# google-research/FirstOrderLp.jl

Hardware: AMD Instinct MI355X
Metric: pdhg_iterations_per_sec (higher is better)
Workload: dtype f64; 1 GPU; random LP m=10000000 n=10000000 nnz=100000000 seed=12345 (BASELINE configs[4]), adaptive step, zero start, no restarts/rescaling; id=configs[4], m=10000000, n=10000000, nnz=100000000, parallelism=single GPU

## Files before the change

firstorderlp.jl_amd/csrc/abi_batch.hpp:

```cpp

struct BatchProduct {
  int rows = 0, grid = 0, slots = 0, long_thr = 0;
  int nlong = 0, nchunks = 0, long_grid = 0, chunk_grid = 0;
  int *long_row = nullptr, *long_cptr = nullptr;
  int2 *chunks = nullptr;
  double *cpart = nullptr;
  double *part = nullptr;
};

struct BatchState {
  int K = 0, shift = 0;
  std::vector<pdhg_handle *> mem;
  BatchProduct PA, PT;
  double *X = nullptr, *Y = nullptr;
  BatchMemberDev *mdev = nullptr, *mhost = nullptr;
  int *act_dev = nullptr, *act_host = nullptr;
  double *res_dev = nullptr, *res_host = nullptr;
  int64_t trials = 0;
};

static void batch_free_product(BatchProduct &P) {
  for (void *p : {(void *)P.long_row, (void *)P.long_cptr, (void *)P.chunks, (void *)P.cpart, (void *)P.part})
    if (p) (void)hipFree(p);
  P = BatchProduct{};
// ... 60 lines not shown
    HIP_TRY(hipMemcpy(P.long_cptr, lcptr.data(), sizeof(int) * lcptr.size(), hipMemcpyHostToDevice));
    HIP_TRY(hipMemcpy(P.chunks, ch.data(), sizeof(int2) * ch.size(), hipMemcpyHostToDevice));
    int rc = alloc_zero(&P.cpart, (int64_t)P.nchunks << shift);
    if (rc) return rc;
  }
  P.slots = P.grid + P.long_grid;
  return 0;
}

static pdhg_handle *batch_of(pdhg_handle *h) { return (h && h->bat) ? h : nullptr; }

static int batch_scale_members(pdhg_handle *h, const double *dv, const double *ev) {
  for (pdhg_handle *m : h->bat->mem) {
    hipLaunchKernelGGL(batch_scale_vectors_kernel, dim3(h->ew_grid_nm), dim3(TPB), 0, h->stream, (int)h->n, (int)h->m, dv, ev,
                       m->c, m->lb, m->ub, m->b);
    m->state_version += 1;
    m->matrix_version += 1;
  }
  HIP_TRY(hipGetLastError());
  return 0;
}

int pdhg_create_batch(pdhg_handle **out, int count, int64_t m, int64_t n, int64_t nnz, const int64_t *colptr,
                      const int64_t *rowval, const double *nzval, int index_base, const double *c, const double *b,
                      const double *lb, const double *ub, int64_t num_equalities, int device_id, void *stream) {
  if (!out) return fail(-1, "out == NULL");
  *out = nullptr;
  if (count < 1 || count > BATCH_MAX) return fail(-1, "pdhg_create_batch: count must be 1.." + std::to_string(BATCH_MAX));
  if (!c || !lb || !ub || (m > 0 && !b)) return fail(-1, "null input array");
  int64_t cap = (int64_t)INT32_MAX - 1;
// ... 175 lines not shown
```

firstorderlp.jl_amd/csrc/abi_measure.hpp:

```cpp


int pdhg_profile_enable(pdhg_handle *h, int enable) {
  int rc0 = check_handle(h);
  if (rc0) return rc0;
  h->profile = enable != 0;
  if (enable) for (int k = 0; k < PDHG_K_COUNT; ++k) { h->prof_count[k] = 0; h->prof_ms[k] = 0.0; }
  return 0;
}

int pdhg_profile_read(pdhg_handle *h, int kernel_id, int64_t *launches, double *total_ms) {
  if (!h || kernel_id < 0 || kernel_id >= PDHG_K_COUNT) return fail(-1, "bad kernel id");
  *launches = h->prof_count[kernel_id];
  *total_ms = h->prof_ms[kernel_id];
  return 0;
}

int64_t pdhg_kernel_algorithmic_bytes(pdhg_handle *h, int kernel_id) {
  if (!h) return -1;
  const int64_t m = h->m, n = h->n, nnz = h->nnz, cn = h->cn;
  const bool group = h->grp != nullptr;
  switch (kernel_id) {
    case PDHG_K_PRIMAL: return 8 * (7 + (h->lazy_accept ? 2 : 0)) * cn;
    case PDHG_K_SPMV_DUAL:
      return nnz * 12 + (m + 1) * 4 + n * 8 + (3 + (h->lazy_accept ? 2 : 0)) * m * 8;
// ... 316 lines not shown

int pdhg_layout_describe(pdhg_handle *h, char *buf, int cap) {
  if (!h) return fail(-1, "null handle");
  std::string out = "{\"A\": " + describe_matrix(h, h->A, MODE_DUAL, 0) + ", \"At\": " + describe_matrix(h, h->At, h->grp ? MODE_PLAIN : MODE_ATY, 1);
  if (h->has_q) out += ", \"Q\": " + describe_matrix(h, h->Q, MODE_PLAIN, 2) + ", \"Qt\": " + describe_matrix(h, h->Qt, MODE_PLAIN, 2);
  if (h->grp && !h->Achunk.empty()) {
    char b[256];
    snprintf(b, sizeof b, ", \"all_gather\": {\"chunks\": %d, \"mode\": \"%s\", \"columns_per_rank_and_chunk\": %lld, \"passes\": [",
             (int)h->Achunk.size(), (h->grp->ag_mode == 1 && h->grp->backend == COMM_RCCL) ? "overlapped with A_p xbar" : "passes behind one all-gather",
             (long long)h->grp->ag_sub);
    out += b;
    for (size_t c = 0; c < h->Achunk.size(); ++c)
      out += (c ? ", " : "") + describe_matrix(h, h->Achunk[c], c + 1 < h->Achunk.size() ? MODE_PLAIN : MODE_DUAL, 0);
    out += "]}";
  }
  const char *tv = getenv("PDHG_TUNE");
  out += std::string(", \"row_order\": \"") + (h->relaxed ? "relaxed" : "strict") + "\", \"timing_at_create\": " + ((tv && tv[0] == '0') ? "false" : "true") + "}";
  if (buf && cap > 0) {
    const size_t k = std::min(out.size(), (size_t)cap - 1);
    memcpy(buf, out.data(), k);
    buf[k] = 0;
  }
  return (int)out.size();
}

int pdhg_layout_info(pdhg_handle *h, int64_t info[16]) {
  if (!h) return fail(-1, "null handle");
  info[12] = (int64_t)h->A.slabs.size(); info[13] = (int64_t)h->At.slabs.size();
  info[14] = (coop_eligible(h) || h->coop_mode == 1) ? 2 : ((graph_eligible(h) || (h->graph_mode == 1 && !h->has_q)) ? 1 : 0);
  info[15] = ((h->A.tiled && h->A.var_tiles) || (!h->A.segs.empty() && h->A.segs.front().tiled && h->A.segs.front().var_tiles) ? 1 : 0) +
// ... 31 lines not shown
```

firstorderlp.jl_amd/csrc/abi_rescale.hpp:

```cpp


static int row_grid(int rows) { return std::max(1, (rows + (TPB / WAVE) - 1) / (TPB / WAVE)); }

struct RescaleTmp {
  double *ev = nullptr, *dv = nullptr, *inv_e = nullptr, *inv_d = nullptr, *cum_e = nullptr, *cum_d = nullptr;
  double *tmp_e = nullptr, *tmp_d = nullptr;
};

extern "C++" {
template <int OP>
static void launch_row_op(pdhg_handle *h, const CsrDev &D, int cols, double pexp, const double *inv_scale, double *out) {
  if (!D.segs.empty()) {
    for (const CsrDev &S : D.segs) launch_row_op<OP>(h, S, cols, pexp, inv_scale ? inv_scale + S.row0 : inv_scale, out + S.row0);
    return;
  }
  hipLaunchKernelGGL(row_op_kernel<OP>, dim3(row_grid(D.rows)), dim3(TPB), 0, h->stream, D.view(), cols, pexp, inv_scale, out,
                     D.long_thr);
  if (D.nlong > 0) {
    hipLaunchKernelGGL(row_op_long_partial_kernel<OP>, dim3(D.nchunks), dim3(TPB), 0, h->stream, D.view(),
                       (const int *)D.chunk_row, (const int *)D.chunk_off, pexp, inv_scale, D.chunk_partial);
    hipLaunchKernelGGL(row_op_long_final_kernel<OP>, dim3(D.long_grid), dim3(TPB), 0, h->stream, D.view(),
                       (const int *)D.long_row, (const int *)D.long_chunk_ptr, D.nlong,
                       (const double *)D.chunk_partial, cols, pexp, out);
  }
// ... 34 lines not shown
  scale_one(h->At, t.inv_e, t.inv_d, 1);
  if (!h->Achunk.empty() && h->grp) {
    DistGroup &g = *h->grp;
    int rc2 = launch_chunk_pack(g, t.inv_d, h->xchunk, 0, g.world, h->n, h->stream);
    if (rc2) return rc2;
    const int64_t W = (int64_t)g.world * g.ag_sub;
    for (size_t c = 0; c < h->Achunk.size(); ++c) scale_one(h->Achunk[c], t.inv_e, h->xchunk + (int64_t)c * W, 0);
  }
  if (h->has_q) {
    scale_one(h->Q, t.inv_d, t.inv_d, 0);
    scale_one(h->Qt, t.inv_d, t.inv_d, 1);
  }
  hipLaunchKernelGGL(resc_apply_vectors_kernel, dim3(h->ew_grid_nm), dim3(TPB), 0, h->stream, n, m, t.dv, t.ev,
                     h->c, h->lb, h->ub, h->b, t.cum_d, t.cum_e);
  HIP_TRY(hipGetLastError());
  if (h->bat) return batch_scale_members(h, t.dv, t.ev);
  return 0;
}

int pdhg_rescale(pdhg_handle *h0, int l_inf_ruiz_iterations, int l2_norm_rescaling,
                 int use_pock_chambolle, double pock_chambolle_alpha,
                 double *constraint_rescaling_out, double *variable_rescaling_out) {
  int rc = check_handle(h0, true, true);
  if (rc) return rc;
  if (h0->owner) return fail(-1, "pdhg_rescale: a batch member shares its batch's matrix: rescale the batch handle");
  if (use_pock_chambolle && !(pock_chambolle_alpha >= 0.0 && pock_chambolle_alpha <= 2.0))
    return fail(-1, "pock_chambolle_alpha must be in [0, 2]");
  const Shards L = shards_of(h0);
  if ((rc = flush_pending(L))) return rc;
  bump_version(L);
// ... 140 lines not shown
```

firstorderlp.jl_amd/csrc/host_shards.hpp:

```cpp


template <typename Src, typename Dst>
int gather_cols_device(const Shards &L, Src src, Dst dst) {
  if (!L.g) {
    pdhg_handle *s = L.p[0];
    if (src(s) != dst(s))
      HIP_TRY(hipMemcpyAsync(dst(s), src(s), sizeof(double) * (size_t)s->n, hipMemcpyDeviceToDevice, s->stream));
    return 0;
  }
  FOR_SHARDS(L, s) {
    if (src(s) != dst(s) && s->cn > 0)
      HIP_TRY(hipMemcpyAsync(dst(s) + s->clo, src(s) + s->clo, sizeof(double) * (size_t)s->cn,
                             hipMemcpyDeviceToDevice, s->stream));
  }
  return dist_all_gather(*L.g, dst, L.g->S);
}

template <typename Src>
int cols_to_host(const Shards &L, Src src, double *host) {
  if (!L.g || L.g->all_local()) {
    FOR_SHARDS(L, s) {
      if (s->cn > 0)
        HIP_TRY(hipMemcpyAsync(host + s->clo, src(s) + s->clo, sizeof(double) * (size_t)s->cn, hipMemcpyDeviceToHost, s->stream));
    }
// ... 433 lines not shown
  CK(alloc_zero(&h->y, m)); CK(alloc_zero(&h->y_next, m));
  CK(alloc_zero(&h->aty, n_alloc + 1)); CK(alloc_zero(&h->aty_next, n_alloc + 1));
  CK(alloc_zero(&h->sum_x, n)); CK(alloc_zero(&h->sum_y, m));
  CK(alloc_zero(&h->tmp_n, n_alloc)); CK(alloc_zero(&h->tmp_m, m));
  h->ew_grid_n = ew_grid(n); h->ew_grid_m = ew_grid(m); h->ew_grid_nm = ew_grid(std::max(n, m));
  h->pAt_stride = std::max(h->At.slots(), h->ew_grid_n);
  CK(alloc_zero(&h->pA, 2 * (int64_t)std::max(h->A.slots(), 1)));
  CK(alloc_zero(&h->pAt, 6 * (int64_t)std::max(h->pAt_stride, 1)));
  CK(alloc_zero(&h->pQ, 2 * (int64_t)h->ew_grid_n));
  CK(alloc_zero(&h->scal_dev, SCAL_MAX));
#undef CK
  hipError_t e = hipHostMalloc((void **)&h->scal_host, sizeof(double) * SCAL_MAX * DIST_MAX_WORLD, hipHostMallocDefault);
  if (e != hipSuccess) return fail((int)e, "hipHostMalloc failed");
  e = hipEventCreate(&h->ev0); if (e == hipSuccess) e = hipEventCreate(&h->ev1);
  if (e != hipSuccess) return fail((int)e, "hipEventCreate failed");
  return 0;
}

int create_shard(pdhg_handle **out, int64_t m, int64_t n, int64_t nnz,
                 const int64_t *colptr, const int64_t *rowval, const double *nzval,
                 int index_base, const double *c, const double *b, const double *lb,
                 const double *ub, int64_t num_equalities, int device_id, void *stream, int64_t n_alloc, int64_t seg_cap) {
  *out = nullptr;
  if (index_base != 0 && index_base != 1) return fail(-1, "index_base must be 0 or 1");
  if (num_equalities < 0 || num_equalities > m) return fail(-1, "num_equalities out of range");
  if (!colptr || !c || !lb || !ub || (m > 0 && !b) || (nnz > 0 && (!rowval || !nzval)))
    return fail(-1, "null input array");
  int ndev = 0;
  HIP_TRY(hipGetDeviceCount(&ndev));
  if (ndev <= 0) return fail(-3, "no HIP device visible");
  int dev = device_id;
// ... 81 lines not shown
  free_csr_dev(h->Q); free_csr_dev(h->Qt);
  for (CsrDev &D : h->Achunk) free_csr_dev(D);
  if (h->chunk_carry) (void)hipFree(h->chunk_carry);
  if (h->xchunk) (void)hipFree(h->xchunk);
  for (hipEvent_t ev : h->ev_ag) if (ev) (void)hipEventDestroy(ev);
  if (h->ev_xbar) (void)hipEventDestroy(h->ev_xbar);
  double *bufs[] = {h->c, h->b, h->lb, h->ub, h->x, h->x_next, h->xbar, h->y, h->y_next,
                    h->aty, h->aty_next, h->sum_x, h->sum_y, h->qx, h->tmp_n, h->tmp_n2,
                    h->tmp_m, h->pA, h->pAt, h->pQ, h->scal_dev, h->scal_all, h->dn_buf, h->dm_buf,
                    h->E, h->Dv, h->c_o, h->b_o, h->lb_o,
                    h->ub_o, h->x_r, h->y_r, h->px_avg, h->py_avg, h->ev_ax, h->ev_aty, h->tr_g,
                    h->tr_dir, h->tr_thr, h->ev_partials, h->ev_cax[0], h->ev_cax[1], h->ev_cax[2],
                    h->ev_caty[0], h->ev_caty[1], h->ev_caty[2], h->ev_cqx[0], h->ev_cqx[1], h->ev_cqx[2],
                    h->ev_qx, h->ev_xg};
  for (double *p : bufs) if (p) (void)hipFree(p);
  graph_destroy(h->tgraph[0]); graph_destroy(h->tgraph[1]);
  if (h->comm_stream) { (void)hipStreamSynchronize(h->comm_stream); (void)hipStreamDestroy(h->comm_stream); }
  for (hipEvent_t ev : h->ev_part) if (ev) (void)hipEventDestroy(ev);
  if (h->ev_comm) (void)hipEventDestroy(h->ev_comm);
  if (h->seq_dev) (void)hipFree(h->seq_dev);
  if (h->gsync) (void)hipFree(h->gsync);
  if (h->tr_sync) (void)hipFree(h->tr_sync);
  if (h->lsync) (void)hipFree(h->lsync);
  if (h->tr_partials) (void)hipFree(h->tr_partials);
  if (h->trb_scratch) (void)hipFree(h->trb_scratch);
  if (h->trb_partials) (void)hipFree(h->trb_partials);
  if (h->coop_trace) (void)hipFree(h->coop_trace);
  if (h->res_host) (void)hipHostFree((void *)h->res_host);
  if (h->scal_host) (void)hipHostFree(h->scal_host);
  if (h->ev_host) (void)hipHostFree(h->ev_host);
// ... 174 lines not shown
```

firstorderlp.jl_amd/csrc/host_trial_graph_build.hpp:

```cpp

bool graph_eligible(pdhg_handle *h) {
  if (h->graph_mode < 0) {
    const char *ev = getenv("PDHG_GRAPH");
    const bool tiled_ok = dev_env("PDHG_GRAPH_TILED") != nullptr;
    bool on = !h->grp && !h->has_q && h->n > 0 && h->A.segs.empty() && h->At.segs.empty() && (tiled_ok || (!h->A.tiled && !h->At.tiled));
    if (ev) on = on && ev[0] != '0';
    h->graph_mode = on ? 1 : 0;
  }
  return h->graph_mode == 1 && !h->has_q && !h->profile;
}

void graph_destroy(pdhg_handle::TrialGraph &G) {
  if (G.exec) (void)hipGraphExecDestroy(G.exec);
  if (G.graph) (void)hipGraphDestroy(G.graph);
  G = pdhg_handle::TrialGraph();
}

struct GraphArgs {
  pdhg_handle *h;
  int n;
  dim3 primal_grid;
  EpiArgs dual_epi;
  GraphArgs(pdhg_handle *h_, double sigma) : h(h_), n((int)h_->n), primal_grid(ew_grid((h_->n + 1) / 2)) {
    dual_epi = dual_epilogue(h, sigma);
// ... 163 lines not shown
    HIP_TRY(graph_set_kernel(G.exec, G.n_dual_long, (const void *)spmv_long_final_kernel<MODE_DUAL>,
                             dim3(A.long_grid), dim3(TPB), (const int *)A.long_row, (const int *)A.long_chunk_ptr,
                             A.nlong, (const double *)A.chunk_partial, dual_epi, A.grid));
  return 0;
}

int graph_build(pdhg_handle *h, pdhg_handle::TrialGraph &G, double tau, double theta, double sigma) {
  graph_destroy(G);
  int rcw = ensure_result_word(h);
  if (rcw) return rcw;
  HIP_TRY(hipGraphCreate(&G.graph, 0));
  GraphArgs a(h, sigma);
  const double *nullq = nullptr;
  HIP_TRY(graph_add_kernel(G.graph, &G.n_primal, {}, (const void *)primal_kernel<false, true>, a.primal_grid, dim3(TPB),
                           a.n, (const double *)h->x, (const double *)h->c, (const double *)h->aty, nullq,
                           (const double *)h->lb, (const double *)h->ub, tau, theta, h->x_next, h->xbar,
                           h->pend_w, h->pend_x ? h->sum_x : (double *)nullptr));
  std::vector<hipGraphNode_t> dual_done, aty_done;
  {
    int rc = graph_add_spmv<MODE_DUAL, 0>(h, G.graph, h->A, h->xbar, a.dual_epi, {G.n_primal}, dual_done, &G.n_dual, &G.n_dual_long);
    if (rc) return rc;
  }
  if (dual_done.empty()) dual_done.push_back(G.n_primal);
  const CsrDev &A = h->A;
  const CsrDev &T = h->At;
  {
    int rc = graph_add_spmv<MODE_ATY, 1>(h, G.graph, T, h->y_next, aty_epilogue(h), dual_done, aty_done, nullptr, nullptr);
    if (rc) return rc;
  }
  if (aty_done.empty()) aty_done = dual_done;
  const FinalSpec sp = trial_final_spec(h, T.slots(), A.slots(), 0, A.slots(), nullptr);
  hipGraphNode_t fin = nullptr;
  HIP_TRY(graph_add_kernel(G.graph, &fin, aty_done, (const void *)final_reduce_host_kernel, dim3(1), dim3(FINAL_TPB), sp,
                           h->seq_dev, h->res_host));
  HIP_TRY(hipGraphInstantiate(&G.exec, G.graph, nullptr, nullptr, 0));
  G.x = h->x; G.y = h->y; G.aty = h->aty;
  G.tau = tau; G.theta = theta; G.sigma = sigma;
  G.add_x = h->pend_x; G.add_wx = h->pend_w;
  G.add_y = h->pend_y; G.add_wy = h->pend_w;
  return 0;
}

int graph_trial(pdhg_handle *h, const TrialArgs &ta, double out[5]) {
  const double tau = ta.step_size / ta.primal_weight, sigma = ta.primal_weight * ta.step_size, theta = ta.theta;
  pdhg_handle::TrialGraph *G = nullptr;
  for (int k = 0; k < 2; ++k)
    if (h->tgraph[k].exec && h->tgraph[k].x == h->x && h->tgraph[k].y == h->y && h->tgraph[k].aty == h->aty)
      G = &h->tgraph[k];
  if (!G) {
    G = !h->tgraph[0].exec ? &h->tgraph[0] : (!h->tgraph[1].exec ? &h->tgraph[1] : &h->tgraph[0]);
    int rc = graph_build(h, *G, tau, theta, sigma);
    if (rc) return rc;
  } else {
    const auto c0 = std::chrono::steady_clock::now();
    GraphArgs a(h, sigma);
    if (G->tau != tau || G->theta != theta || G->add_x != h->pend_x || (h->pend_x && G->add_wx != h->pend_w)) {
      const double *nullq = nullptr;
      HIP_TRY(graph_set_kernel(G->exec, G->n_primal, (const void *)primal_kernel<false, true>, a.primal_grid, dim3(TPB),
                               a.n, (const double *)h->x, (const double *)h->c, (const double *)h->aty, nullq,
                               (const double *)h->lb, (const double *)h->ub, tau, theta, h->x_next, h->xbar,
                               h->pend_w, h->pend_x ? h->sum_x : (double *)nullptr));
      G->tau = tau; G->theta = theta;
      G->add_x = h->pend_x; G->add_wx = h->pend_w;
    }
    if (G->sigma != sigma || G->add_y != h->pend_y || (h->pend_y && G->add_wy != h->pend_w)) {
      int rc = graph_set_dual(h, *G, a.dual_epi);
      if (rc) return rc;
      G->sigma = sigma;
      G->add_y = h->pend_y; G->add_wy = h->pend_w;
    }
    h->t_set += std::chrono::duration<double>(std::chrono::steady_clock::now() - c0).count();
  }
  h->seq_expected += 1;
  const auto c1 = std::chrono::steady_clock::now();
  HIP_TRY(hipGraphLaunch(G->exec, h->stream));
#ifdef PDHG_PROBE_GRAPH_TWICE
  HIP_TRY(hipGraphLaunch(G->exec, h->stream));
// ... 54 lines not shown
```

firstorderlp.jl_amd/csrc/pdhg_hip.hip:

```cpp
#include <hip/hip_runtime.h>
#include <dlfcn.h>

#include <algorithm>
#include <atomic>
#include <chrono>
#include <condition_variable>
#include <functional>
#include <cmath>
#include <cstdint>
#include <cstdio>
#include <cstdlib>
#include <cstring>
#include <string>
#include <mutex>
#include <thread>
#include <vector>

#include "pdhg_hip.h"

#include "common.hpp"
#include "spmv_kernels.hpp"
#include "sj_kernels.hpp"
#include "vector_kernels.hpp"
#include "grid_sync.hpp"
// ... 13 lines not shown
struct pdhg_handle {
  int device = 0;
  hipStream_t stream = nullptr;
  bool own_stream = false;
  int64_t m = 0, n = 0, nnz = 0, num_eq = 0;
  bool remap = true;
  bool relaxed = true;

  CsrDev A;
  CsrDev At;
  bool has_q = false;
  CsrDev Q;
  CsrDev Qt;

  double *c = nullptr, *b = nullptr, *lb = nullptr, *ub = nullptr;
  double *x = nullptr, *x_next = nullptr, *xbar = nullptr;
  double *y = nullptr, *y_next = nullptr;
  double *aty = nullptr, *aty_next = nullptr;
  double *sum_x = nullptr, *sum_y = nullptr;
  double *qx = nullptr, *tmp_n = nullptr, *tmp_n2 = nullptr, *tmp_m = nullptr;
  int64_t sum_x_count = 0, sum_y_count = 0;
  bool pend_x = false, pend_y = false, lazy_accept = true;
  double pend_w = 0.0;
  double sum_x_weights = 0.0, sum_y_weights = 0.0;

  double *pA = nullptr;
  double *pAt = nullptr;
  double *pQ = nullptr;
  int pAt_stride = 0;
  int ew_grid_n = 1, ew_grid_m = 1, ew_grid_nm = 1;
// ... 50 lines not shown
  double *xchunk = nullptr;
  std::vector<hipEvent_t> ev_ag;
  hipEvent_t ev_xbar = nullptr;
  double *dn_buf = nullptr;
  double *dm_buf = nullptr;
  double *scal_dev = nullptr, *scal_all = nullptr, *scal_host = nullptr;
  double *ev_host = nullptr;
  unsigned long long ev_seq = 0;

  struct TrialGraph {
    hipGraph_t graph = nullptr;
    hipGraphExec_t exec = nullptr;
    hipGraphNode_t n_primal = nullptr, n_dual = nullptr, n_dual_long = nullptr;
    const double *x = nullptr, *y = nullptr, *aty = nullptr;
    double tau = 0.0, theta = 0.0, sigma = 0.0;
    bool add_x = false, add_y = false;
    double add_wx = 0.0, add_wy = 0.0;
  } tgraph[2];
  int coop_mode = -1;
  int coop_grid = 0;
  unsigned coop_nxcd = 0;
  unsigned coop_xcd_cnt[8] = {0};
  unsigned long long coop_launches = 0, coop_epoch = 0;
  int local_mode = -1;
  GridSync *lsync = nullptr;
  unsigned long long local_epoch = 0;
  long local_launches = 0;
  GridSync *gsync = nullptr;
  unsigned long long *coop_trace = nullptr;
  int graph_mode = -1;
// ... 229 lines not shown
  e.out = out;
  if (with_long && D.nlong > 0) {
    hipLaunchKernelGGL(spmv_long_partial_kernel<1>, dim3(D.nchunks), dim3(TPB), 0, h->stream,
                       D.view(), xin, D.chunk_row, D.chunk_off, D.chunk_partial);
    hipLaunchKernelGGL(spmv_long_final_kernel<MODE_PLAIN>, dim3(D.long_grid), dim3(TPB), 0, h->stream,
                       D.long_row, D.long_chunk_ptr, D.nlong, D.chunk_partial, e, D.grid);
  }
  if (g1 > g0) {
    int rc = launch_tiled<MODE_PLAIN>(h, D, xin, e, g0, g1);
    if (rc) return rc;
  }
  HIP_TRY(hipGetLastError());
  return 0;
}

int launch_primal(pdhg_handle *h, double tau, double theta, bool write_xbar) {
  ProfScope ps(h, PDHG_K_PRIMAL);
  if (h->has_q) {
    EpiArgs e{};
    e.out = h->qx;
    int rc = launch_spmv<MODE_PLAIN, 2>(h, h->Q, h->x, e);
    if (rc) return rc;
  }
  const int n = (int)h->cn;
  const int64_t o = h->clo;
  const int grid = ew_grid((h->cn + 1) / 2);
#define PK(HQ, WX)                                                                           \
  hipLaunchKernelGGL((primal_kernel<HQ, WX>), dim3(grid), dim3(TPB), 0, h->stream, n,        \
                     h->x + o, h->c + o, h->aty + o, h->has_q ? h->qx + o : nullptr, h->lb + o, h->ub + o, tau, theta, \
                     h->x_next + o, h->xbar + o, h->pend_w, h->pend_x ? h->sum_x + o : nullptr)
  if (h->has_q) { if (write_xbar) PK(true, true); else PK(true, false); }
  else          { if (write_xbar) PK(false, true); else PK(false, false); }
#undef PK
  HIP_TRY(hipGetLastError());
  h->pend_x = false;
  return 0;
}

int launch_xbar(pdhg_handle *h, double theta) {
  const int64_t o = h->clo;
  hipLaunchKernelGGL(xbar_kernel, dim3(ew_grid(h->cn)), dim3(TPB), 0, h->stream, (int)h->cn, h->x + o, h->x_next + o,
                     theta, h->xbar + o);
  HIP_TRY(hipGetLastError());
  return 0;
// ... 258 lines not shown
```

firstorderlp.jl_amd/csrc/trial_kernel.hpp:

```cpp
#pragma once

namespace {

#ifndef PDHG_TRIAL_WAVES_PER_EU
#define PDHG_TRIAL_WAVES_PER_EU 4
#endif
#ifndef PDHG_TRIAL_PIPE
#define PDHG_TRIAL_PIPE true
#endif
#ifndef PDHG_STEPS_LP_BATCH
#define PDHG_STEPS_LP_BATCH 8
#endif

struct TrialProduct {
  CsrView M;
  const int2 *blks;
  int nblk, per_xcd, grid, remap;
  int nchunks, nlong, long_grid;
  const int *chunk_row, *chunk_off, *chunk_lidx;
  double *chunk_partial;
  const int *long_row, *long_chunk_ptr;
  unsigned long long *long_ticket;
  const double *xin;
  EpiArgs e;
// ... 107 lines not shown
template <bool COH>
__global__ __launch_bounds__(TPB, PDHG_TRIAL_WAVES_PER_EU) void trial_kernel(TrialKernelArgs a) {
  __shared__ double prod[BLOCK_NNZ];
  __shared__ double red[6][TPB / WAVE];
  const int w = blockIdx.x, nwg = gridDim.x;
#define PDHG_STAMP(k) do { if (a.trace && threadIdx.x == 0) a.trace[(size_t)w * 8 + (k)] = wall_clock64(); } while (0)
  PDHG_STAMP(0);
  Prefetched f;
  unsigned long long epoch = a.epoch;
  if (a.has_q && !a.xbar_only) {
    f.kind = 0;
    product_phase<MODE_PLAIN, COH>(a.Qx, a.Qx.xin, a.Qx.e, a.Qx.uses, a.relaxed, f, prod, red);
    grid_barrier(a.sync, ++epoch, a.nxcd, a.xcd_cnt);
  }
  if (a.xbar_only) xbar_body(a.n, a.x, a.x_next, a.theta, a.xbar, w, nwg);
  else if (a.has_q) primal_body<true, true>(a.n, a.x, a.c, a.aty, a.qx, a.lb, a.ub, a.tau, a.theta, a.x_next, a.xbar, a.avg_w, a.sum_x, w, nwg);
  else primal_body<false, true, COH>(a.n, a.x, a.c, a.aty, nullptr, a.lb, a.ub, a.tau, a.theta, a.x_next, a.xbar, a.avg_w, a.sum_x, w, nwg);
  if (a.has_q) diff_pairs_body(a.n, a.x_next, a.x, a.dx, w, nwg);
  product_prefetch(a.A, f);
  PDHG_STAMP(1);
  grid_barrier(a.sync, ++epoch, a.nxcd, a.xcd_cnt);
  PDHG_STAMP(2);
  product_phase<MODE_DUAL, COH>(a.A, a.A.xin, a.A.e, a.A.uses, a.relaxed, f, prod, red);
  if (a.has_q) {
    Prefetched none;
    none.kind = 0;
    product_phase<MODE_PLAIN, COH>(a.Qtdx, a.Qtdx.xin, a.Qtdx.e, a.Qtdx.uses, a.relaxed, none, prod, red);
  }
  product_prefetch(a.T, f);
  PDHG_STAMP(3);
  grid_barrier(a.sync, ++epoch, a.nxcd, a.xcd_cnt);
  PDHG_STAMP(4);
// ... 81 lines not shown
  __syncthreads();
  while (steps < a.n_steps && (trials < a.max_trials || mid) && trials < a.table_len) {
    const double step = s_st[0], pend_w = s_st[2];
#define PDHG_STAMP(k) do { if (a.trace && threadIdx.x == 0) a.trace[(size_t)w * 8 + (k)] = wall_clock64(); } while (0)
    PDHG_STAMP(0);
    double *x = flip ? a.xb : a.xa, *xn = flip ? a.xa : a.xb;
    double *y = flip ? a.yb : a.ya, *yn = flip ? a.ya : a.yb;
    double *aty = flip ? a.atyb : a.atya, *atyn = flip ? a.atya : a.atyb;
    const double tau = step / a.primal_weight, sigma = a.primal_weight * step;
    unsigned long long err_pref = 0;
    double pw_r = 0.0, pw_g = 0.0;
    if (threadIdx.x == 0) {
      err_pref = __hip_atomic_load(&a.sync->error[0], __ATOMIC_RELAXED, __HIP_MEMORY_SCOPE_AGENT);
      pw_r = a.pow_red[trials]; pw_g = a.pow_growth[trials];
    }
    primal_body<false, true, true>(a.n, x, a.c, aty, nullptr, a.lb, a.ub, tau, 1.0, xn, a.xbar, pend_w,
                                   pend ? a.sum_x : nullptr, w, nwg);
    product_prefetch(a.A, f, w, nwg);
    if (threadIdx.x == 0) { s_pow[0] = pw_r; s_pow[1] = pw_g; }
    PDHG_STAMP(1);
    if (local) grid_barrier_local(a.sync, ++epoch, a.local_home, (unsigned long long)a.local_g, err_pref);
    else grid_barrier(a.sync, ++epoch, a.nxcd, a.xcd_cnt, err_pref);
    PDHG_STAMP(2);
    if (threadIdx.x == 0) err_pref = __hip_atomic_load(&a.sync->error[0], __ATOMIC_RELAXED, __HIP_MEMORY_SCOPE_AGENT);
    {
      EpiArgs e{};
      e.y = y; e.b = a.b; e.y_next = yn; e.sigma = sigma; e.num_eq = a.num_eq;
      e.partials = a.pA; e.stride = a.pA_slots; e.lo_offset = a.pA_slots;
      if (pend) { e.sum_y = a.sum_y; e.avg_w = pend_w; }
      product_phase<MODE_DUAL, true>(a.A, a.xbar, e, a.uses_a + (unsigned long long)trials, a.relaxed, f, prod, red, w, nwg);
    }
// ... 101 lines not shown
```

firstorderlp.jl_amd/csrc/vector_kernels.hpp:

```cpp
#pragma once

namespace {


template <bool HAS_Q, bool WRITE_XBAR>
__device__ __forceinline__ void primal_one(double x, double c, double aty,
                                           double qx, double lb, double ub,
                                           double tau, double theta, double &xn,
                                           double &xb) {
  const double q = HAS_Q ? qx : 0.0;
  const double t0 = q + c;
  const double g = t0 - aty;
  const double t1 = tau * g;
  double v = x - t1;
  v = jl_min(ub, jl_max(lb, v));
  xn = v;
  if (WRITE_XBAR) {
    const double d = v - x;
    const double t2 = theta * d;
    xb = v + t2;
  }
}

template <bool HAS_Q, bool WRITE_XBAR, bool COH = false>
__device__ __forceinline__ void primal_body(
    int n, const double *x, const double *c, const double *aty, const double *qx,
    const double *lb, const double *ub, double tau, double theta, double *x_next, double *xbar,
    double avg_w, double *sum_x, int bid, int nb) {
  const int npair = n >> 1;
  const int stride = nb * TPB;
  for (int p = bid * TPB + threadIdx.x; p < npair; p += stride) {
    const double2 xv = reinterpret_cast<const double2 *>(x)[p];
    if (sum_x) {
      double2 sv = reinterpret_cast<double2 *>(sum_x)[p];
      const double t0 = xv.x * avg_w, t1 = xv.y * avg_w;
      sv.x = sv.x + t0;
      sv.y = sv.y + t1;
      reinterpret_cast<double2 *>(sum_x)[p] = sv;
    }
    const double2 cv = reinterpret_cast<const double2 *>(c)[p];
    double2 av;
    if (COH) { av.x = ldc<true>(aty + 2 * p); av.y = ldc<true>(aty + 2 * p + 1); }
    else av = reinterpret_cast<const double2 *>(aty)[p];
    const double2 lv = reinterpret_cast<const double2 *>(lb)[p];
    const double2 uv = reinterpret_cast<const double2 *>(ub)[p];
    double2 qv = {0.0, 0.0};
    if (HAS_Q) qv = reinterpret_cast<const double2 *>(qx)[p];
    double2 xn, xb;
    primal_one<HAS_Q, WRITE_XBAR>(xv.x, cv.x, av.x, qv.x, lv.x, uv.x, tau, theta, xn.x, xb.x);
    primal_one<HAS_Q, WRITE_XBAR>(xv.y, cv.y, av.y, qv.y, lv.y, uv.y, tau, theta, xn.y, xb.y);
    {
      reinterpret_cast<double2 *>(x_next)[p] = xn;
      if (WRITE_XBAR) reinterpret_cast<double2 *>(xbar)[p] = xb;
    }
  }
  if ((n & 1) && bid == 0 && threadIdx.x == 0) {
    const int j = n - 1;
    double xn, xb;
    if (sum_x) {
      const double t = x[j] * avg_w;
      sum_x[j] = sum_x[j] + t;
    }
    primal_one<HAS_Q, WRITE_XBAR>(x[j], c[j], ldc<COH>(aty + j), HAS_Q ? qx[j] : 0.0, lb[j], ub[j], tau, theta, xn, xb);
    x_next[j] = xn;
    if (WRITE_XBAR) xbar[j] = xb;
  }
}

template <bool HAS_Q, bool WRITE_XBAR>
__global__ __launch_bounds__(TPB) void primal_kernel(
    int n, const double *__restrict__ x, const double *__restrict__ c,
    const double *__restrict__ aty, const double *__restrict__ qx,
    const double *__restrict__ lb, const double *__restrict__ ub, double tau,
    double theta, double *__restrict__ x_next, double *__restrict__ xbar,
    double avg_w, double *__restrict__ sum_x) {
  primal_body<HAS_Q, WRITE_XBAR>(n, x, c, aty, qx, lb, ub, tau, theta, x_next, xbar, avg_w, sum_x, blockIdx.x, gridDim.x);
}

__device__ __forceinline__ void xbar_body(int n, const double *x, const double *x_next, double theta, double *xbar,
                                          int bid, int nb) {
  const int stride = nb * TPB;
  for (int j = bid * TPB + threadIdx.x; j < n; j += stride) {
    const double v = x_next[j];
    const double d = v - x[j];
    const double t = theta * d;
    xbar[j] = v + t;
  }
}
__global__ __launch_bounds__(TPB) void xbar_kernel(int n, const double *__restrict__ x,
                                                   const double *__restrict__ x_next,
                                                   double theta, double *__restrict__ xbar) {
// ... 200 lines not shown
```

firstorderlp.jl_amd/engine.py:

```python
import ctypes

import numpy as np

from . import _lib

_dp = ctypes.POINTER(ctypes.c_double)
_ip = ctypes.POINTER(ctypes.c_int64)
_int_p = ctypes.POINTER(ctypes.c_int)


def _d(a):
    return np.ascontiguousarray(a, dtype=np.float64)


def _i(a):
    return np.ascontiguousarray(a, dtype=np.int64)


def _pd(a):
    return None if a is None else a.ctypes.data_as(_dp)


def _pi(a):
    return a.ctypes.data_as(_ip)
# ... 373 lines not shown
        out["A_segments"] = (out["var_tiles"] >> 8) & 255
        out["At_segments"] = (out["var_tiles"] >> 16) & 255
        out["group_coop_trials"] = (out["var_tiles"] >> 24) & 65535
        out["group_coop_fallbacks"] = (out["var_tiles"] >> 40) & 255
        out["tr_coop_calls"] = (out["var_tiles"] >> 48) & 16383
        out["var_tiles"] &= 3
        try:
            desc = self.layout_describe()
            for k in ("A", "At", "Q", "Qt"):
                if k in desc:
                    sj = desc[k].get("sliced_jagged")
                    if k in ("Q", "Qt"):
                        out[k + "_sj"] = 1 if sj else 0
                    out[k + "_sj_wide"] = 1 if sj and sj["slices_per_wave"] > 1 else 0
                    out[k + "_sj_hub_rows"] = sj["hub_rows"] if sj else 0
        except Exception:
            pass
        for k in ("A", "At"):
            out[k + "_tile_shift"] = max(1, (out[k + "_tile_cols"] - 1).bit_length()) if out[k + "_tile_cols"] else 0
        return out


class _MemberEngine(HipPdhgEngine):

    def close(self):
        self._h = None


class _MemberOwner:

# ... 26 lines not shown
```

Measured before the change: 605.2 iterations/s.

## Compress lb/ub into constant or sparse-exception form for the primal kernel

Adds a census at setup and after rescaling that finds the most common value in each bound vector. If that value covers at least three quarters of the entries, the vector is stored either as a single constant or as a default plus a bitmask, per-block prefix counts and a packed exception array. The standalone primal kernel and the trial graph's primal node now take bound views and dispatch on the mode, so they skip streaming two dense n-length f64 vectors each iteration. The cooperative trial kernel still reads dense bounds. The change adds setup synchronisations and a popcount-based lookup for sparse mode.

```diff
diff --git a/firstorderlp.jl_amd/csrc/abi_batch.hpp b/firstorderlp.jl_amd/csrc/abi_batch.hpp
--- a/firstorderlp.jl_amd/csrc/abi_batch.hpp
+++ b/firstorderlp.jl_amd/csrc/abi_batch.hpp
@@ -98,6 +98,8 @@
   for (pdhg_handle *m : h->bat->mem) {
     hipLaunchKernelGGL(batch_scale_vectors_kernel, dim3(h->ew_grid_nm), dim3(TPB), 0, h->stream, (int)h->n, (int)h->m, dv, ev,
                        m->c, m->lb, m->ub, m->b);
+    HIP_TRY(hipGetLastError());
+    if (int rcb = bounds_rebuild(m)) return rcb;
     m->state_version += 1;
     m->matrix_version += 1;
   }
diff --git a/firstorderlp.jl_amd/csrc/abi_measure.hpp b/firstorderlp.jl_amd/csrc/abi_measure.hpp
--- a/firstorderlp.jl_amd/csrc/abi_measure.hpp
+++ b/firstorderlp.jl_amd/csrc/abi_measure.hpp
@@ -354,6 +354,13 @@
       out += (c ? ", " : "") + describe_matrix(h, h->Achunk[c], c + 1 < h->Achunk.size() ? MODE_PLAIN : MODE_DUAL, 0);
     out += "]}";
   }
+  {
+    static const char *mode_name[3] = {"dense", "const", "sparse"};
+    char b[256];
+    snprintf(b, sizeof b, ", \"bounds\": {\"lb\": {\"mode\": \"%s\", \"exceptions\": %lld}, \"ub\": {\"mode\": \"%s\", \"exceptions\": %lld}}",
+             mode_name[h->bnd[0].mode], (long long)h->bnd[0].nexc, mode_name[h->bnd[1].mode], (long long)h->bnd[1].nexc);
+    out += b;
+  }
   const char *tv = getenv("PDHG_TUNE");
   out += std::string(", \"row_order\": \"") + (h->relaxed ? "relaxed" : "strict") + "\", \"timing_at_create\": " + ((tv && tv[0] == '0') ? "false" : "true") + "}";
   if (buf && cap > 0) {
diff --git a/firstorderlp.jl_amd/csrc/abi_rescale.hpp b/firstorderlp.jl_amd/csrc/abi_rescale.hpp
--- a/firstorderlp.jl_amd/csrc/abi_rescale.hpp
+++ b/firstorderlp.jl_amd/csrc/abi_rescale.hpp
@@ -72,6 +72,7 @@
   hipLaunchKernelGGL(resc_apply_vectors_kernel, dim3(h->ew_grid_nm), dim3(TPB), 0, h->stream, n, m, t.dv, t.ev,
                      h->c, h->lb, h->ub, h->b, t.cum_d, t.cum_e);
   HIP_TRY(hipGetLastError());
+  if (int rcb = bounds_rebuild(h)) return rcb;
   if (h->bat) return batch_scale_members(h, t.dv, t.ev);
   return 0;
 }
diff --git a/firstorderlp.jl_amd/csrc/host_shards.hpp b/firstorderlp.jl_amd/csrc/host_shards.hpp
--- a/firstorderlp.jl_amd/csrc/host_shards.hpp
+++ b/firstorderlp.jl_amd/csrc/host_shards.hpp
@@ -471,7 +471,7 @@
   if (e != hipSuccess) return fail((int)e, "hipHostMalloc failed");
   e = hipEventCreate(&h->ev0); if (e == hipSuccess) e = hipEventCreate(&h->ev1);
   if (e != hipSuccess) return fail((int)e, "hipEventCreate failed");
-  return 0;
+  return bounds_rebuild(h);
 }
 
 int create_shard(pdhg_handle **out, int64_t m, int64_t n, int64_t nnz,
@@ -583,6 +583,7 @@
                     h->ev_caty[0], h->ev_caty[1], h->ev_caty[2], h->ev_cqx[0], h->ev_cqx[1], h->ev_cqx[2],
                     h->ev_qx, h->ev_xg};
   for (double *p : bufs) if (p) (void)hipFree(p);
+  bounds_free(h);
   graph_destroy(h->tgraph[0]); graph_destroy(h->tgraph[1]);
   if (h->comm_stream) { (void)hipStreamSynchronize(h->comm_stream); (void)hipStreamDestroy(h->comm_stream); }
   for (hipEvent_t ev : h->ev_part) if (ev) (void)hipEventDestroy(ev);
diff --git a/firstorderlp.jl_amd/csrc/host_trial_graph_build.hpp b/firstorderlp.jl_amd/csrc/host_trial_graph_build.hpp
--- a/firstorderlp.jl_amd/csrc/host_trial_graph_build.hpp
+++ b/firstorderlp.jl_amd/csrc/host_trial_graph_build.hpp
@@ -201,7 +201,7 @@
   const double *nullq = nullptr;
   HIP_TRY(graph_add_kernel(G.graph, &G.n_primal, {}, (const void *)primal_kernel<false, true>, a.primal_grid, dim3(TPB),
                            a.n, (const double *)h->x, (const double *)h->c, (const double *)h->aty, nullq,
-                           (const double *)h->lb, (const double *)h->ub, tau, theta, h->x_next, h->xbar,
+                           bound_view(h, 0), bound_view(h, 1), tau, theta, h->x_next, h->xbar,
                            h->pend_w, h->pend_x ? h->sum_x : (double *)nullptr));
   std::vector<hipGraphNode_t> dual_done, aty_done;
   {
@@ -223,6 +223,7 @@
   HIP_TRY(hipGraphInstantiate(&G.exec, G.graph, nullptr, nullptr, 0));
   G.x = h->x; G.y = h->y; G.aty = h->aty;
   G.tau = tau; G.theta = theta; G.sigma = sigma;
+  G.bounds_version = h->bounds_version;
   G.add_x = h->pend_x; G.add_wx = h->pend_w;
   G.add_y = h->pend_y; G.add_wy = h->pend_w;
   return 0;
@@ -241,13 +242,14 @@
   } else {
     const auto c0 = std::chrono::steady_clock::now();
     GraphArgs a(h, sigma);
-    if (G->tau != tau || G->theta != theta || G->add_x != h->pend_x || (h->pend_x && G->add_wx != h->pend_w)) {
+    if (G->tau != tau || G->theta != theta || G->add_x != h->pend_x || (h->pend_x && G->add_wx != h->pend_w) ||
+        G->bounds_version != h->bounds_version) {
       const double *nullq = nullptr;
       HIP_TRY(graph_set_kernel(G->exec, G->n_primal, (const void *)primal_kernel<false, true>, a.primal_grid, dim3(TPB),
                                a.n, (const double *)h->x, (const double *)h->c, (const double *)h->aty, nullq,
-                               (const double *)h->lb, (const double *)h->ub, tau, theta, h->x_next, h->xbar,
+                               bound_view(h, 0), bound_view(h, 1), tau, theta, h->x_next, h->xbar,
                                h->pend_w, h->pend_x ? h->sum_x : (double *)nullptr));
-      G->tau = tau; G->theta = theta;
+      G->tau = tau; G->theta = theta; G->bounds_version = h->bounds_version;
       G->add_x = h->pend_x; G->add_wx = h->pend_w;
     }
     if (G->sigma != sigma || G->add_y != h->pend_y || (h->pend_y && G->add_wy != h->pend_w)) {
diff --git a/firstorderlp.jl_amd/csrc/pdhg_hip.hip b/firstorderlp.jl_amd/csrc/pdhg_hip.hip
--- a/firstorderlp.jl_amd/csrc/pdhg_hip.hip
+++ b/firstorderlp.jl_amd/csrc/pdhg_hip.hip
@@ -51,6 +51,15 @@
   CsrDev Qt;
 
   double *c = nullptr, *b = nullptr, *lb = nullptr, *ub = nullptr;
+  struct BoundsDev {
+    int mode = BND_DENSE;
+    double def = 0.0;
+    int64_t nexc = 0;
+    unsigned long long *mask = nullptr;
+    int *blk = nullptr;
+    double *exc = nullptr;
+  } bnd[2];
+  uint64_t bounds_version = 0;
   double *x = nullptr, *x_next = nullptr, *xbar = nullptr;
   double *y = nullptr, *y_next = nullptr;
   double *aty = nullptr, *aty_next = nullptr;
@@ -131,6 +140,7 @@
     hipGraphNode_t n_primal = nullptr, n_dual = nullptr, n_dual_long = nullptr;
     const double *x = nullptr, *y = nullptr, *aty = nullptr;
     double tau = 0.0, theta = 0.0, sigma = 0.0;
+    uint64_t bounds_version = 0;
     bool add_x = false, add_y = false;
     double add_wx = 0.0, add_wy = 0.0;
   } tgraph[2];
@@ -390,6 +400,73 @@
   return 0;
 }
 
+void bounds_free(pdhg_handle *h) {
+  for (pdhg_handle::BoundsDev &B : h->bnd) {
+    for (void *p : {(void *)B.mask, (void *)B.blk, (void *)B.exc}) if (p) (void)hipFree(p);
+    B = pdhg_handle::BoundsDev{};
+  }
+}
+
+int bounds_rebuild(pdhg_handle *h) {
+  HIP_TRY(hipStreamSynchronize(h->stream));
+  bounds_free(h);
+  h->bounds_version += 1;
+  const int n = (int)h->n;
+  const char *ev = dev_env("PDHG_BOUNDS");
+  if (n <= 0 || (ev && !strcmp(ev, "dense"))) return 0;
+  unsigned *cnt = nullptr;
+  HIP_TRY(hipMalloc((void **)&cnt, sizeof(unsigned) * 8));
+  auto body = [&]() -> int {
+    const double *src[2] = {h->lb, h->ub};
+    HIP_TRY(hipMemsetAsync(cnt, 0, sizeof(unsigned) * 8, h->stream));
+    for (int k = 0; k < 2; ++k)
+      hipLaunchKernelGGL(bound_census_kernel, dim3(h->ew_grid_n), dim3(TPB), 0, h->stream, n, src[k], cnt + 4 * k);
+    HIP_TRY(hipGetLastError());
+    unsigned hc[8];
+    uint64_t first[2];
+    HIP_TRY(hipMemcpyAsync(hc, cnt, sizeof hc, hipMemcpyDeviceToHost, h->stream));
+    for (int k = 0; k < 2; ++k) HIP_TRY(hipMemcpyAsync(&first[k], src[k], sizeof(uint64_t), hipMemcpyDeviceToHost, h->stream));
+    HIP_TRY(hipStreamSynchronize(h->stream));
+    for (int k = 0; k < 2; ++k) {
+      pdhg_handle::BoundsDev &B = h->bnd[k];
+      const uint64_t cand[4] = {first[k], 0x7FF0000000000000ull, 0xFFF0000000000000ull, 0ull};
+      int best = 0;
+      for (int q = 1; q < 4; ++q) if (hc[4 * k + q] > hc[4 * k + best]) best = q;
+      const int64_t nexc = (int64_t)n - (int64_t)hc[4 * k + best];
+      if (4 * nexc > (int64_t)n) continue;
+      memcpy(&B.def, &cand[best], sizeof(double));
+      B.nexc = nexc;
+      if (nexc == 0) { B.mode = BND_CONST; continue; }
+      const int nblk = (n + BND_BLOCK - 1) / BND_BLOCK;
+      HIP_TRY(hipMalloc((void **)&B.mask, sizeof(unsigned long long) * 2 * (size_t)nblk));
+      HIP_TRY(hipMalloc((void **)&B.blk, sizeof(int) * (size_t)nblk));
+      HIP_TRY(hipMalloc((void **)&B.exc, sizeof(double) * (size_t)nexc));
+      hipLaunchKernelGGL(bound_mask_kernel, dim3(ew_grid((int64_t)nblk * WAVE)), dim3(TPB), 0, h->stream, n, src[k],
+                         (unsigned long long)cand[best], B.mask, B.blk);
+      HIP_TRY(hipGetLastError());
+      int rc = device_exclusive_scan(B.blk, B.blk, nblk, nullptr, h->stream);
+      if (rc) return rc;
+      hipLaunchKernelGGL(bound_pack_kernel, dim3(h->ew_grid_n), dim3(TPB), 0, h->stream, n, src[k],
+                         (const unsigned long long *)B.mask, (const int *)B.blk, B.exc);
+      HIP_TRY(hipGetLastError());
+      B.mode = BND_SPARSE;
+    }
+    HIP_TRY(hipStreamSynchronize(h->stream));
+    return 0;
+  };
+  const int rc = body();
+  (void)hipFree(cnt);
+  if (rc) bounds_free(h);
+  return rc;
+}
+
+BoundView bound_view(const pdhg_handle *h, int k) {
+  const pdhg_handle::BoundsDev &B = h->bnd[k];
+  BoundView v = bound_dense(k == 0 ? h->lb : h->ub);
+  v.mask = B.mask; v.blk = B.blk; v.exc = B.exc; v.def = B.def; v.mode = B.mode;
+  return v;
+}
+
 int launch_primal(pdhg_handle *h, double tau, double theta, bool write_xbar) {
   ProfScope ps(h, PDHG_K_PRIMAL);
   if (h->has_q) {
@@ -401,9 +478,11 @@
   const int n = (int)h->cn;
   const int64_t o = h->clo;
   const int grid = ew_grid((h->cn + 1) / 2);
+  const bool whole = o == 0 && h->cn == h->n;
+  const BoundView lbv = whole ? bound_view(h, 0) : bound_dense(h->lb + o), ubv = whole ? bound_view(h, 1) : bound_dense(h->ub + o);
 #define PK(HQ, WX)                                                                           \
   hipLaunchKernelGGL((primal_kernel<HQ, WX>), dim3(grid), dim3(TPB), 0, h->stream, n,        \
-                     h->x + o, h->c + o, h->aty + o, h->has_q ? h->qx + o : nullptr, h->lb + o, h->ub + o, tau, theta, \
+                     h->x + o, h->c + o, h->aty + o, h->has_q ? h->qx + o : nullptr, lbv, ubv, tau, theta, \
                      h->x_next + o, h->xbar + o, h->pend_w, h->pend_x ? h->sum_x + o : nullptr)
   if (h->has_q) { if (write_xbar) PK(true, true); else PK(true, false); }
   else          { if (write_xbar) PK(false, true); else PK(false, false); }
diff --git a/firstorderlp.jl_amd/csrc/trial_kernel.hpp b/firstorderlp.jl_amd/csrc/trial_kernel.hpp
--- a/firstorderlp.jl_amd/csrc/trial_kernel.hpp
+++ b/firstorderlp.jl_amd/csrc/trial_kernel.hpp
@@ -145,8 +145,8 @@
     grid_barrier(a.sync, ++epoch, a.nxcd, a.xcd_cnt);
   }
   if (a.xbar_only) xbar_body(a.n, a.x, a.x_next, a.theta, a.xbar, w, nwg);
-  else if (a.has_q) primal_body<true, true>(a.n, a.x, a.c, a.aty, a.qx, a.lb, a.ub, a.tau, a.theta, a.x_next, a.xbar, a.avg_w, a.sum_x, w, nwg);
-  else primal_body<false, true, COH>(a.n, a.x, a.c, a.aty, nullptr, a.lb, a.ub, a.tau, a.theta, a.x_next, a.xbar, a.avg_w, a.sum_x, w, nwg);
+  else if (a.has_q) primal_body<true, true>(a.n, a.x, a.c, a.aty, a.qx, bound_dense(a.lb), bound_dense(a.ub), a.tau, a.theta, a.x_next, a.xbar, a.avg_w, a.sum_x, w, nwg);
+  else primal_body<false, true, COH>(a.n, a.x, a.c, a.aty, nullptr, bound_dense(a.lb), bound_dense(a.ub), a.tau, a.theta, a.x_next, a.xbar, a.avg_w, a.sum_x, w, nwg);
   if (a.has_q) diff_pairs_body(a.n, a.x_next, a.x, a.dx, w, nwg);
   product_prefetch(a.A, f);
   PDHG_STAMP(1);
@@ -258,7 +258,7 @@
       err_pref = __hip_atomic_load(&a.sync->error[0], __ATOMIC_RELAXED, __HIP_MEMORY_SCOPE_AGENT);
       pw_r = a.pow_red[trials]; pw_g = a.pow_growth[trials];
     }
-    primal_body<false, true, true>(a.n, x, a.c, aty, nullptr, a.lb, a.ub, tau, 1.0, xn, a.xbar, pend_w,
+    primal_body<false, true, true>(a.n, x, a.c, aty, nullptr, bound_dense(a.lb), bound_dense(a.ub), tau, 1.0, xn, a.xbar, pend_w,
                                    pend ? a.sum_x : nullptr, w, nwg);
     product_prefetch(a.A, f, w, nwg);
     if (threadIdx.x == 0) { s_pow[0] = pw_r; s_pow[1] = pw_g; }
diff --git a/firstorderlp.jl_amd/csrc/vector_kernels.hpp b/firstorderlp.jl_amd/csrc/vector_kernels.hpp
--- a/firstorderlp.jl_amd/csrc/vector_kernels.hpp
+++ b/firstorderlp.jl_amd/csrc/vector_kernels.hpp
@@ -22,10 +22,55 @@
   }
 }
 
-template <bool HAS_Q, bool WRITE_XBAR, bool COH = false>
+enum { BND_DENSE = 0, BND_CONST = 1, BND_SPARSE = 2 };
+constexpr int BND_BLOCK = 2 * WAVE;
+struct BoundView {
+  const double *dense;
+  const unsigned long long *mask;
+  const int *blk;
+  const double *exc;
+  double def;
+  int mode;
+};
+__host__ __device__ inline BoundView bound_dense(const double *p) { return BoundView{p, nullptr, nullptr, nullptr, 0.0, BND_DENSE}; }
+
+template <int BM>
+__device__ __forceinline__ double2 bound_pair(const BoundView &b, int p) {
+  if (BM == BND_DENSE) return reinterpret_cast<const double2 *>(b.dense)[p];
+  double2 r = {b.def, b.def};
+  if (BM == BND_SPARSE) {
+    const int blk = p >> 6, l = p & 63;
+    const ulonglong2 w = reinterpret_cast<const ulonglong2 *>(b.mask)[blk];
+    const int base = b.blk[blk];
+    const unsigned long long mine = l < 32 ? w.x : w.y;
+    const int sh = 2 * (l & 31);
+    const unsigned bits = (unsigned)(mine >> sh) & 3u;
+    if (bits) {
+      const int rank = __popcll(mine & ((1ull << sh) - 1ull)) + (l < 32 ? 0 : __popcll(w.x));
+      const double *e = b.exc + base + rank;
+      if (bits & 1u) r.x = e[0];
+      if (bits & 2u) r.y = e[bits & 1u];
+    }
+  }
+  return r;
+}
+__device__ __forceinline__ double bound_at(const BoundView &b, int j) {
+  if (b.mode == BND_DENSE) return b.dense[j];
+  if (b.mode == BND_SPARSE) {
+    const int wd = j >> 6, bit = j & 63;
+    const unsigned long long w = b.mask[wd];
+    if ((w >> bit) & 1ull) {
+      const int rank = __popcll(w & ((1ull << bit) - 1ull)) + ((wd & 1) ? __popcll(b.mask[wd - 1]) : 0);
+      return b.exc[b.blk[j / BND_BLOCK] + rank];
+    }
+  }
+  return b.def;
+}
+
+template <bool HAS_Q, bool WRITE_XBAR, bool COH = false, int LBM = BND_DENSE, int UBM = BND_DENSE>
 __device__ __forceinline__ void primal_body(
     int n, const double *x, const double *c, const double *aty, const double *qx,
-    const double *lb, const double *ub, double tau, double theta, double *x_next, double *xbar,
+    const BoundView &lb, const BoundView &ub, double tau, double theta, double *x_next, double *xbar,
     double avg_w, double *sum_x, int bid, int nb) {
   const int npair = n >> 1;
   const int stride = nb * TPB;
@@ -42,8 +87,8 @@
     double2 av;
     if (COH) { av.x = ldc<true>(aty + 2 * p); av.y = ldc<true>(aty + 2 * p + 1); }
     else av = reinterpret_cast<const double2 *>(aty)[p];
-    const double2 lv = reinterpret_cast<const double2 *>(lb)[p];
-    const double2 uv = reinterpret_cast<const double2 *>(ub)[p];
+    const double2 lv = bound_pair<LBM>(lb, p);
+    const double2 uv = bound_pair<UBM>(ub, p);
     double2 qv = {0.0, 0.0};
     if (HAS_Q) qv = reinterpret_cast<const double2 *>(qx)[p];
     double2 xn, xb;
@@ -61,7 +106,7 @@
       const double t = x[j] * avg_w;
       sum_x[j] = sum_x[j] + t;
     }
-    primal_one<HAS_Q, WRITE_XBAR>(x[j], c[j], ldc<COH>(aty + j), HAS_Q ? qx[j] : 0.0, lb[j], ub[j], tau, theta, xn, xb);
+    primal_one<HAS_Q, WRITE_XBAR>(x[j], c[j], ldc<COH>(aty + j), HAS_Q ? qx[j] : 0.0, bound_at(lb, j), bound_at(ub, j), tau, theta, xn, xb);
     x_next[j] = xn;
     if (WRITE_XBAR) xbar[j] = xb;
   }
@@ -71,10 +116,71 @@
 __global__ __launch_bounds__(TPB) void primal_kernel(
     int n, const double *__restrict__ x, const double *__restrict__ c,
     const double *__restrict__ aty, const double *__restrict__ qx,
-    const double *__restrict__ lb, const double *__restrict__ ub, double tau,
+    BoundView lb, BoundView ub, double tau,
     double theta, double *__restrict__ x_next, double *__restrict__ xbar,
     double avg_w, double *__restrict__ sum_x) {
-  primal_body<HAS_Q, WRITE_XBAR>(n, x, c, aty, qx, lb, ub, tau, theta, x_next, xbar, avg_w, sum_x, blockIdx.x, gridDim.x);
+#define PDHG_PB(L, U)                                                                                                   \
+  primal_body<HAS_Q, WRITE_XBAR, false, L, U>(n, x, c, aty, qx, lb, ub, tau, theta, x_next, xbar, avg_w, sum_x, blockIdx.x, gridDim.x)
+  switch (lb.mode * 3 + ub.mode) {
+    case BND_DENSE * 3 + BND_CONST: PDHG_PB(BND_DENSE, BND_CONST); break;
+    case BND_DENSE * 3 + BND_SPARSE: PDHG_PB(BND_DENSE, BND_SPARSE); break;
+    case BND_CONST * 3 + BND_DENSE: PDHG_PB(BND_CONST, BND_DENSE); break;
+    case BND_CONST * 3 + BND_CONST: PDHG_PB(BND_CONST, BND_CONST); break;
+    case BND_CONST * 3 + BND_SPARSE: PDHG_PB(BND_CONST, BND_SPARSE); break;
+    case BND_SPARSE * 3 + BND_DENSE: PDHG_PB(BND_SPARSE, BND_DENSE); break;
+    case BND_SPARSE * 3 + BND_CONST: PDHG_PB(BND_SPARSE, BND_CONST); break;
+    case BND_SPARSE * 3 + BND_SPARSE: PDHG_PB(BND_SPARSE, BND_SPARSE); break;
+    default: PDHG_PB(BND_DENSE, BND_DENSE); break;
+  }
+#undef PDHG_PB
+}
+
+__global__ __launch_bounds__(TPB) void bound_census_kernel(int n, const double *__restrict__ v, unsigned *__restrict__ cnt) {
+  const int lane = threadIdx.x & (WAVE - 1);
+  const int gw = (blockIdx.x * TPB + threadIdx.x) / WAVE, nw = gridDim.x * (TPB / WAVE);
+  const unsigned long long cand[4] = {(unsigned long long)__double_as_longlong(v[0]), 0x7FF0000000000000ull,
+                                      0xFFF0000000000000ull, 0ull};
+  unsigned c[4] = {0u, 0u, 0u, 0u};
+  for (int64_t base = (int64_t)gw * WAVE; base < n; base += (int64_t)nw * WAVE) {
+    const int64_t j = base + lane;
+    const bool ok = j < n;
+    const unsigned long long b = ok ? (unsigned long long)__double_as_longlong(v[j]) : 0ull;
+#pragma unroll
+    for (int q = 0; q < 4; ++q) c[q] += (unsigned)__popcll(__ballot(ok && b == cand[q]));
+  }
+  if (lane == 0) {
+#pragma unroll
+    for (int q = 0; q < 4; ++q) if (c[q]) atomicAdd(cnt + q, c[q]);
+  }
+}
+__global__ __launch_bounds__(TPB) void bound_mask_kernel(int n, const double *__restrict__ v, unsigned long long def,
+                                                         unsigned long long *__restrict__ mask, int *__restrict__ cnt) {
+  const int lane = threadIdx.x & (WAVE - 1);
+  const int gw = (blockIdx.x * TPB + threadIdx.x) / WAVE, nw = gridDim.x * (TPB / WAVE);
+  const int nblk = (n + BND_BLOCK - 1) / BND_BLOCK;
+  for (int b = gw; b < nblk; b += nw) {
+    const int64_t j0 = (int64_t)b * BND_BLOCK + lane, j1 = j0 + WAVE;
+    const unsigned long long w0 = __ballot(j0 < n && (unsigned long long)__double_as_longlong(v[j0 < n ? j0 : 0]) != def);
+    const unsigned long long w1 = __ballot(j1 < n && (unsigned long long)__double_as_longlong(v[j1 < n ? j1 : 0]) != def);
+    if (lane == 0) {
+      mask[2 * (size_t)b] = w0;
+      mask[2 * (size_t)b + 1] = w1;
+      cnt[b] = __popcll(w0) + __popcll(w1);
+    }
+  }
+}
+__global__ __launch_bounds__(TPB) void bound_pack_kernel(int n, const double *__restrict__ v,
+                                                         const unsigned long long *__restrict__ mask,
+                                                         const int *__restrict__ blk, double *__restrict__ exc) {
+  const int stride = gridDim.x * TPB;
+  for (int j = blockIdx.x * TPB + threadIdx.x; j < n; j += stride) {
+    const int wd = j >> 6, bit = j & 63;
+    const unsigned long long w = mask[wd];
+    if ((w >> bit) & 1ull) {
+      const int rank = __popcll(w & ((1ull << bit) - 1ull)) + ((wd & 1) ? __popcll(mask[wd - 1]) : 0);
+      exc[blk[j / BND_BLOCK] + rank] = v[j];
+    }
+  }
 }
 
 __device__ __forceinline__ void xbar_body(int n, const double *x, const double *x_next, double theta, double *xbar,
diff --git a/firstorderlp.jl_amd/engine.py b/firstorderlp.jl_amd/engine.py
--- a/firstorderlp.jl_amd/engine.py
+++ b/firstorderlp.jl_amd/engine.py
@@ -411,6 +411,9 @@
                         out[k + "_sj"] = 1 if sj else 0
                     out[k + "_sj_wide"] = 1 if sj and sj["slices_per_wave"] > 1 else 0
                     out[k + "_sj_hub_rows"] = sj["hub_rows"] if sj else 0
+            for k in ("lb", "ub"):
+                out[k + "_mode"] = desc["bounds"][k]["mode"]
+                out[k + "_exceptions"] = desc["bounds"][k]["exceptions"]
         except Exception:
             pass
         for k in ("A", "At"):
```

After: 612.2 iterations/s (median of 6 runs). 1.2% higher.
